# DecodeGenetics/BamQC

Measured on AMD Instinct MI355X. Metric: BAM records/sec (and GB/s vs HBM roofline), 150 bp PE, 1/2/4/8 MI355X, higher is better.
Workload: dtype u8/u32/u64 integer

## Files before the change

bamqc_amd/csrc/bqc_pipeline.cpp:

```cpp
#include "bqc_ctx.h"

#include <algorithm>
#include <chrono>
#include <climits>
#include <cstdlib>
#include <cstring>

#include "../host/parallel.h"

extern "C" {
void bqc_launch_reads_chunks(const DevBatch&, const StateLayout&, uint64_t*, const DevRefs&, uint32_t*, uint32_t grid, uint32_t fast_table, hipStream_t);
void bqc_launch_nm_extra(const DevBatch&, const StateLayout&, uint64_t*, const DevRefs&, uint32_t*, hipStream_t);
void bqc_launch_long(const DevBatch&, const StateLayout&, uint64_t*, const DevRefs&, uint32_t*, uint32_t*, uint32_t max_len_ub, uint32_t max_read_len, uint32_t, uint32_t, uint32_t* t8rows, uint32_t* t8_used, uint32_t t8_lane, uint32_t* cyc_tiles, uint32_t* cyc_used, uint32_t slot_cap, hipStream_t);
uint32_t bqc_long_slots(uint32_t max_len_ub, uint32_t max_read_len, uint32_t n_chunks_ub, uint32_t n_cu);
void bqc_launch_cov(const DevBatch&, const StateLayout&, uint64_t*, uint32_t* carry, uint32_t* parity, const uint8_t* lane_mask, uint8_t* started,
                    const uint8_t* started_after, uint32_t n_lanes, hipStream_t);
void bqc_launch_add_words(uint64_t* state, const uint64_t* idx, const uint64_t* val, uint32_t n, hipStream_t);
void bqc_launch_or_bytes(uint8_t* dst, const uint8_t* src, uint32_t n, hipStream_t);
void bqc_launch_short(const DevBatch&, const StateLayout&, uint64_t*, const DevRefs&, uint32_t*, uint32_t grid, uint32_t* t8rows, uint32_t* t8_used, hipStream_t);
uint32_t bqc_short_parts();
void bqc_launch_t8_fold(const uint32_t* t8rows, const uint32_t* t8_used, uint32_t n_slots, const StateLayout&, uint64_t* state, uint32_t lane, hipStream_t);
void bqc_launch_err_merge(ErrRec* dst, const ErrRec* src, hipStream_t);
void bqc_launch_cov_final(const StateLayout&, uint64_t*, const uint32_t* carry, const uint32_t* parity, const uint8_t* started, const uint8_t* sel, uint32_t count_start, hipStream_t);
}
// ... 338 lines not shown
    Carver cv;
    cv.take(256);
    m.h2d_begin = cv.off;
    const size_t cb[13] = {2 * n, n, n, 4 * n, 4 * n, 4 * n, 4 * n, 4 * n, 4 * n, 2 * n, H.seq_bytes, H.qual_bytes, 4 * H.cigar_words};
    for (int k = 0; k < 13; ++k) { m.col_bytes[k] = in_place ? 0 : cb[k]; m.o_col[k] = cv.take(in_place ? 0 : cb[k] + (k >= 10 ? 512 : 0)); }
    m.o_xr = cv.take(4ull * b->n_nm_extra); m.o_xv = cv.take(4ull * b->n_nm_extra);
    m.o_cov_in = cv.take(in_place ? 0 : sizeof(CovEntry) * n);
    m.o_order = cv.take(H.multi_lane ? 4 * n : 0);
    m.o_sws = cv.take(sizeof(SuperWindow) * H.sws.size());
    m.o_stretch = cv.take(sizeof(Stretch) * H.stretches.size());
    m.o_tiles = cv.take(sizeof(CovTile) * H.tiles.size());
    m.o_mask = cv.take(nl); m.o_started = cv.take(nl);
    m.o_aidx = cv.take(8 * H.add_idx.size()); m.o_aval = cv.take(8 * H.add_val.size());
    m.h2d_end = cv.off;
    const uint64_t nblk = (n + 1023) / 1024, n_sw = H.sws.size(), n_st = H.stretches.size();
    const uint64_t perm_cap = 3 * n + H.cigar_words + 128 * (n_sw + n_st + 1);
    const uint64_t cf_cap = (2 * n + 128 * n_sw) / 256 + H.cigar_words / 256 + 4 * n_st + 16;
    const uint64_t cs_cap = H.n_slow / BQC_CHUNK_READS + n_st + 4;
    const uint64_t cx_cap = H.cigar_words / 2 + 1;
    if (perm_cap > 0xFFFFFFF0ull) return bqc_fail(c, BQC_ERR_ARG, "batch too large (split the batch)");
    const size_t o_flag2 = cv.take(2 * n), o_soff = cv.take(4 * n), o_qoff = cv.take(4 * n), o_cgoff = cv.take(4 * n), o_cov = cv.take(sizeof(CovEntry) * n),
                 o_covx = cv.take(sizeof(CovExtra) * cx_cap), o_cls = cv.take(2 * n), o_segs = cv.take(sizeof(TripSeg) * (H.cigar_words + 1)),
                 o_perm = cv.take(4 * perm_cap), o_cf = cv.take(sizeof(Chunk) * cf_cap), o_cs = cv.take(sizeof(Chunk) * cs_cap),
                 o_desc = cv.take(sizeof(BatchDesc)), o_err = cv.take(sizeof(ErrRec)), o_cursave = cv.take(8), o_bsz = cv.take(24 * nblk), o_btgt = cv.take(8 * nblk),
                 o_bmf = cv.take(8 * nblk), o_swc = cv.take(sizeof(SwCounts) * n_sw), o_swp = cv.take(sizeof(SwPlan) * n_sw),
                 o_rsum = cv.take(H.n_slow ? 12 * n : 0), o_otmp = cv.take(order_on_device && H.multi_lane ? 4 * lane_order_tmp_words((uint32_t)n, nl) : 0);
    const size_t need = cv.off + 256;
    if (m.dcap < need) {
        if (m.dmem) { (void)hipFree(m.dmem); m.dmem = nullptr; m.dcap = 0; }
        if (from_pool)
            for (size_t k = 0; k < c->pool.size(); ++k)
                if (c->pool[k].second >= need && c->pool[k].second <= 2 * need + (64u << 20)) {
                    m.dmem = c->pool[k].first; m.dcap = c->pool[k].second;
                    c->pool.erase(c->pool.begin() + k);
                    break;
                }
        if (!m.dmem) {
            const size_t cap = need + need / 8;
            const hipError_t he = hipMalloc(&m.dmem, cap);
            if (he != hipSuccess) { m.dmem = nullptr; return bqc_fail(c, BQC_ERR_DEVICE, "hipMalloc(%zu) failed: %s", cap, hipGetErrorString(he)); }
            m.dcap = cap;
        }
    }
    char* base = (char*)m.dmem;
    DevBatch& d = m.d;
    d = DevBatch{};
    d.n_reads = (uint32_t)n;
// ... 9 lines not shown
    d.chunks = (const Chunk*)(base + o_cs); d.chunks_fast = (const Chunk*)(base + o_cf);
    d.desc = (const BatchDesc*)(base + o_desc);
    d.nm_extra_read = (const uint32_t*)(base + m.o_xr); d.nm_extra_val = (const int32_t*)(base + m.o_xv); d.n_nm_extra = b->n_nm_extra;
    d.cov = (const CovEntry*)(base + o_cov); d.cov_extra = (const CovExtra*)(base + o_covx);
    d.cov_tiles = (const CovTile*)(base + m.o_tiles); d.n_cov_tiles = (uint32_t)H.tiles.size();
    d.segs = (const TripSeg*)(base + o_segs);
    PrepArgs& p = m.prep;
    p = PrepArgs{};
    p.n = (uint32_t)n; p.n_lanes = nl; p.max_read_len = c->opt.max_read_len; p.no_fast = c->no_fast ? 1u : 0u; p.replay = 0;
    p.flag_in = (const uint16_t*)(base + m.o_col[0]); p.mapq = d.mapq; p.lane = d.lane; p.rid = d.rid; p.pos = d.pos; p.as_ = d.as_;
    p.l_seq = d.l_seq; p.n_cigar = d.n_cigar; p.qual = d.qual; p.cigar = d.cigar;
    p.cov_in = (const CovEntry*)(base + m.o_cov_in); p.order = d.order;
    p.sws = (const SuperWindow*)(base + m.o_sws); p.n_sw = (uint32_t)n_sw;
    p.stretches = (const Stretch*)(base + m.o_stretch); p.n_stretch = (uint32_t)n_st;
    p.fasta_index = c->d_fasta_index;
    p.flag_out = (uint16_t*)(base + o_flag2); p.seq_off = (uint32_t*)(base + o_soff); p.qual_off = (uint32_t*)(base + o_qoff);
    p.cigar_off = (uint32_t*)(base + o_cgoff); p.cov_out = (CovEntry*)(base + o_cov); p.cov_extra = (CovExtra*)(base + o_covx);
    p.cov_extra_cap = (uint32_t)std::min<uint64_t>(cx_cap, 0xFFFFFFFFull); p.cls = (uint16_t*)(base + o_cls); p.segs = (TripSeg*)(base + o_segs);
    p.perm = (uint32_t*)(base + o_perm); p.perm_cap = (uint32_t)perm_cap;
    p.chunks_fast = (Chunk*)(base + o_cf); p.chunks_fast_cap = (uint32_t)cf_cap;
    p.chunks_slow = (Chunk*)(base + o_cs); p.chunks_slow_cap = (uint32_t)cs_cap;
    p.desc = (BatchDesc*)(base + o_desc); p.err = (ErrRec*)(base + o_err);
    p.cursor = c->d_cursor; p.cursor_save = (int32_t*)(base + o_cursave);
    p.blk_sizes = (unsigned long long*)(base + o_bsz); p.blk_tgt = (uint32_t*)(base + o_btgt); p.blk_maxfast = (uint32_t*)(base + o_bmf);
    p.sw_counts = (SwCounts*)(base + o_swc); p.sw_plan = (SwPlan*)(base + o_swp);
    m.d_lane_mask = (uint8_t*)(base + m.o_mask); m.d_started_after = (uint8_t*)(base + m.o_started);
    m.d_add_idx = (uint64_t*)(base + m.o_aidx); m.d_add_val = (uint64_t*)(base + m.o_aval); m.n_add = (uint32_t)H.add_idx.size();
    m.d_rsum = H.n_slow ? (uint32_t*)(base + o_rsum) : nullptr;
    m.d_order_tmp = order_on_device && H.multi_lane ? (uint32_t*)(base + o_otmp) : nullptr;
    m.d_err = p.err;
    m.algo_bytes = 48ull * n + H.seq_bytes + H.qual_bytes + 4 * H.cigar_words;
    m.n_slow = H.n_slow; m.max_len_slow = H.max_len_slow; m.n_chunks_slow_ub = (uint32_t)cs_cap; m.t8_lane = H.t8_lane;
    m.lane_bits[0] = m.lane_bits[1] = m.lane_bits[2] = m.lane_bits[3] = 0;
    for (size_t l = 0; l < H.lane_count.size() && l < 256; ++l) if (H.lane_count[l]) m.lane_bits[l >> 6] |= 1ull << (l & 63);
    if (in_place) {
        d.mapq = b->mapq; d.lane = b->lane; d.rid = b->rid; d.pos = b->pos; d.tlen = b->tlen; d.nm = b->nm; d.as_ = b->as; d.l_seq = b->l_seq; d.n_cigar = b->n_cigar;
        d.seq = b->seq; d.qual = b->qual; d.cigar = b->cigar;
        p.flag_in = b->flag; p.mapq = d.mapq; p.lane = d.lane; p.rid = d.rid; p.pos = d.pos; p.as_ = d.as_; p.l_seq = d.l_seq; p.n_cigar = d.n_cigar; p.qual = d.qual; p.cigar = d.cigar;
        p.cov_in = in_place;
    }
    m.processed = false;
    return 0;
}

static void fill_tables(const BatchMem& m, const bqc_batch* b, const HostPass& H, char* img, size_t img_begin , bool anchors_on_device = false)
{
    auto at = [&](size_t off) { return img + (off - img_begin); };
// ... 665 lines not shown
```

bamqc_amd/csrc/k_prep.hip:

```cpp
#include <algorithm>
#include "kernels_common.h"
#include "prep.h"

#define PR_THREADS 256
#define PR_PER_THREAD 4
#define PR_BLOCK (PR_THREADS * PR_PER_THREAD)

__device__ __forceinline__ uint32_t wave_scan_incl_max(uint32_t v)
{
    v = max(v, (uint32_t)__builtin_amdgcn_update_dpp(0, (int)v, 0x111, 0xF, 0xF, true));
    v = max(v, (uint32_t)__builtin_amdgcn_update_dpp(0, (int)v, 0x112, 0xF, 0xF, true));
    v = max(v, (uint32_t)__builtin_amdgcn_update_dpp(0, (int)v, 0x114, 0xF, 0xF, true));
    v = max(v, (uint32_t)__builtin_amdgcn_update_dpp(0, (int)v, 0x118, 0xF, 0xF, true));
    v = max(v, (uint32_t)__builtin_amdgcn_update_dpp(0, (int)v, 0x142, 0xA, 0xF, false));
    v = max(v, (uint32_t)__builtin_amdgcn_update_dpp(0, (int)v, 0x143, 0xC, 0xF, false));
    return v;
}
__device__ __forceinline__ uint32_t block_scan_excl(uint32_t v, uint32_t* sh, uint32_t* total)
{
    const uint32_t inc = wave_scan_incl(v), w = threadIdx.x >> 6, nw = blockDim.x >> 6;
    block_sync();
    if (lane_id() == WAVE - 1) sh[w] = inc;
    block_sync();
    uint32_t base = 0, tot = 0;
    for (uint32_t k = 0; k < nw; ++k) { const uint32_t x = sh[k]; if (k < w) base += x; tot += x; }
    *total = tot;
    return base + inc - v;
}
__device__ __forceinline__ uint32_t block_scan_excl_max(uint32_t v, uint32_t* sh, uint32_t* total)
{
    const uint32_t inc = wave_scan_incl_max(v), w = threadIdx.x >> 6, nw = blockDim.x >> 6;
    block_sync();
    if (lane_id() == WAVE - 1) sh[w] = inc;
    block_sync();
    uint32_t base = 0, tot = 0;
    for (uint32_t k = 0; k < nw; ++k) { const uint32_t x = sh[k]; if (k < w) base = max(base, x); tot = max(tot, x); }
    *total = tot;
    const uint32_t prev = (uint32_t)__builtin_amdgcn_update_dpp(0, (int)inc, 0x138 , 0xF, 0xF, true);
    return max(base, prev);
}
__device__ __forceinline__ void err_key(ErrRec* e, uint32_t read, uint32_t order)
{
    atomicMin(&e->first_key, ((unsigned long long)read << 3) | order);
}

__global__ __launch_bounds__(PR_THREADS) void k_prep_sizes(PrepArgs a)
{
    __shared__ unsigned long long sh[3 * (PR_THREADS / 64)];
    if (blockIdx.x == 0 && threadIdx.x == 0) {
        a.err->first_key = BQC_ERRKEY_NONE; a.err->flags = 0; a.err->aux0 = a.err->aux1 = 0;
        a.desc->n_cov_extra = 0;
        if (a.pend_extra_n) *a.pend_extra_n = 0;
        if (a.replay) *a.cursor = *a.cursor_save; else *a.cursor_save = *a.cursor;
    }
    for (uint32_t k = blockIdx.x * PR_THREADS + threadIdx.x; k < a.n_sw; k += gridDim.x * PR_THREADS) a.sw_counts[k] = SwCounts{0, 0, 0, 0};
    const uint32_t b0 = blockIdx.x * PR_BLOCK;
    unsigned long long s1 = 0, s2 = 0, s3 = 0;
#pragma unroll
    for (int j = 0; j < PR_PER_THREAD; ++j) {
        const uint32_t i = b0 + j * PR_THREADS + threadIdx.x;
        if (i < a.n) { const uint32_t L = a.l_seq[i]; s1 += (L + 1) / 2; s2 += L; s3 += a.n_cigar[i]; }
    }
#pragma unroll
    for (int o = 32; o > 0; o >>= 1) { s1 += __shfl_xor(s1, o); s2 += __shfl_xor(s2, o); s3 += __shfl_xor(s3, o); }
    if (lane_id() == 0) { const uint32_t w = threadIdx.x >> 6; sh[3 * w] = s1; sh[3 * w + 1] = s2; sh[3 * w + 2] = s3; }
    block_sync();
    if (threadIdx.x < 3) {
        unsigned long long t = 0;
        for (uint32_t w = 0; w < PR_THREADS / 64; ++w) t += sh[3 * w + threadIdx.x];
        a.blk_sizes[3ull * blockIdx.x + threadIdx.x] = t;
    }
}

__global__ __launch_bounds__(1024) void k_prep_scan(PrepArgs a)
{
    __shared__ unsigned long long sh[3 * 1024];
    const uint32_t nblk = (a.n + PR_BLOCK - 1) / PR_BLOCK;
    const uint32_t per = (nblk + blockDim.x - 1) / blockDim.x;
    const uint32_t lo = min(nblk, threadIdx.x * per), hi = min(nblk, lo + per);
    unsigned long long t[3] = {0, 0, 0};
    for (uint32_t b = lo; b < hi; ++b)
        for (int k = 0; k < 3; ++k) t[k] += a.blk_sizes[3ull * b + k];
    for (int k = 0; k < 3; ++k) sh[3 * threadIdx.x + k] = t[k];
    block_sync();
    for (uint32_t d = 1; d < blockDim.x; d <<= 1) {
        unsigned long long v[3] = {0, 0, 0};
        if (threadIdx.x >= d) for (int k = 0; k < 3; ++k) v[k] = sh[3 * (threadIdx.x - d) + k];
        block_sync();
        for (int k = 0; k < 3; ++k) sh[3 * threadIdx.x + k] += v[k];
        block_sync();
    }
    unsigned long long run[3];
    for (int k = 0; k < 3; ++k) run[k] = sh[3 * threadIdx.x + k] - t[k];
    for (uint32_t b = lo; b < hi; ++b) {
        bool over = false;
        for (int k = 0; k < 3; ++k) {
            const unsigned long long s = a.blk_sizes[3ull * b + k];
            a.blk_sizes[3ull * b + k] = run[k];
            run[k] += s;
            over |= run[k] > 0xFFFFFFFFull;
        }
        if (over) err_key(a.err, b * PR_BLOCK, 3);
    }
}

struct CigarView {
    uint32_t w[4];
    const uint32_t* cg;
    __device__ __forceinline__ uint32_t at(uint32_t k) const
    {
        if (k < 4u) return k == 0u ? w[0] : k == 1u ? w[1] : k == 2u ? w[2] : w[3];
        return cg[k];
    }
};
__device__ __forceinline__ int triplet_eligible(uint32_t flag, uint32_t mapq, int32_t as, const CigarView& cv, uint32_t ncig)
{
    if (!(flag & 0x1) || !(flag & 0x2) || (flag & 0x4) || (flag & 0x8) || (flag & 0x100)) return 0;
    if (mapq < 60) return 0;
    if (as == BQC_AS_ABSENT || as < 0) return -1;
    if (as < 50) return 0;
    uint32_t clipped = 0;
    for (uint32_t k = 0; k < ncig; ++k) {
        const uint32_t wd = cv.at(k), op = wd & 15u;
        if (op == 4u || op == 5u) clipped += wd >> 4;
    }
// ... 91 lines not shown
                        a.segs[co + nseg] = TripSeg{i, (int32_t)posv, (uint32_t)ia | ((uint32_t)ib << 8), 0};
                        ++nseg;
                    }
                    rp += nn; cpos += nn;
                }
            }
        }
    }
    o.flag = flag;
    o.ce = ce;
    o.cls = ((fast ? ((flag & 0x40u) ? 0u : 1u) : 2u) << 8) | nseg;
    return o;
}

#ifndef PR_WAVES_PER_EU
#define PR_WAVES_PER_EU 4
#endif
__global__ __launch_bounds__(PR_THREADS) __attribute__((amdgpu_waves_per_eu(PR_WAVES_PER_EU, PR_WAVES_PER_EU))) void k_prep_reads(PrepArgs a, DevRefs refs)
{
    __shared__ uint32_t sh[2 * (PR_THREADS / 64)];
    __shared__ uint32_t red[8];
    const uint32_t i0 = blockIdx.x * PR_BLOCK + 4u * threadIdx.x;
    const unsigned long long gs = a.blk_sizes[3ull * blockIdx.x], gq = a.blk_sizes[3ull * blockIdx.x + 1], gc = a.blk_sizes[3ull * blockIdx.x + 2];
    if (threadIdx.x < 8) red[threadIdx.x] = threadIdx.x == 0 ? 0xFFFFFFFFu : 0u;
    ReadIn in[4];
    const uint32_t nlive = i0 >= a.n ? 0u : min(4u, a.n - i0);
    if (nlive == 4u) {
        const uint4 vl = *(const uint4*)(a.l_seq + i0);
        const uint2 vc = *(const uint2*)(a.n_cigar + i0), vf = *(const uint2*)(a.flag_in + i0);
        const uint32_t vlane = *(const uint32_t*)(a.lane + i0), vmq = *(const uint32_t*)(a.mapq + i0);
        const int4 vr = *(const int4*)(a.rid + i0), vp = *(const int4*)(a.pos + i0), va = *(const int4*)(a.as_ + i0);
        const uint4 c01 = *(const uint4*)(a.cov_in + i0), c23 = *(const uint4*)(a.cov_in + i0 + 2);
        const uint32_t Ls[4] = {vl.x, vl.y, vl.z, vl.w}, ncs[4] = {vc.x & 0xFFFFu, vc.x >> 16, vc.y & 0xFFFFu, vc.y >> 16};
        const uint32_t fs[4] = {vf.x & 0xFFFFu, vf.x >> 16, vf.y & 0xFFFFu, vf.y >> 16};
        const int32_t rs[4] = {vr.x, vr.y, vr.z, vr.w}, ps[4] = {vp.x, vp.y, vp.z, vp.w}, as[4] = {va.x, va.y, va.z, va.w};
        const CovEntry cs[4] = {{c01.x, c01.y}, {c01.z, c01.w}, {c23.x, c23.y}, {c23.z, c23.w}};
#pragma unroll
        for (int j = 0; j < 4; ++j) in[j] = ReadIn{Ls[j], ncs[j], fs[j], (vlane >> (8 * j)) & 0xFFu, (vmq >> (8 * j)) & 0xFFu, rs[j], ps[j], as[j], cs[j]};
    } else {
#pragma unroll
        for (int j = 0; j < 4; ++j) {
            in[j] = ReadIn{0, 0, 0x900u, 0, 0, -1, 0, 0, CovEntry{BQC_COV_NONE, 0}};
            if ((uint32_t)j < nlive) { const uint32_t i = i0 + j; in[j] = ReadIn{a.l_seq[i], a.n_cigar[i], a.flag_in[i], a.lane[i], a.mapq[i], a.rid[i], a.pos[i], a.as_[i], a.cov_in[i]}; }
        }
    }
    uint32_t ls[4], lq[4], lc[4], ts = 0, tq = 0, tc = 0;
#pragma unroll
    for (int j = 0; j < 4; ++j) { ls[j] = ts; lq[j] = tq; lc[j] = tc; ts += (in[j].L + 1) / 2; tq += in[j].L; tc += in[j].nc; }
    uint32_t tot;
    const unsigned long long bs = gs + block_scan_excl(ts, sh, &tot), bq = gq + block_scan_excl(tq, sh, &tot), bc = gc + block_scan_excl(tc, sh, &tot);
    ReadOut out[4];
    CigarView cv[4];
    bool ref_loaded[4];
    int32_t target[4];
    unsigned long long cos[4];
    bool oks[4];
#pragma unroll
    for (int j = 0; j < 4; ++j) {
        const unsigned long long so = bs + ls[j], qo = bq + lq[j], co = bc + lc[j];
        cos[j] = co;
        oks[j] = so + (in[j].L + 1) / 2 <= 0xFFFFFFFFull && qo + in[j].L <= 0xFFFFFFFFull && co + in[j].nc <= 0xFFFFFFFFull;
        const bool live = (uint32_t)j < nlive && oks[j];
        cv[j].cg = a.cigar + (uint32_t)co;
#pragma unroll
        for (uint32_t k = 0; k < 4u; ++k) cv[j].w[k] = live && k < in[j].nc ? cv[j].cg[k] : 0u;
        const int32_t rid = in[j].rid;
        const bool rid_ok = (uint32_t)j < nlive && rid >= 0 && (uint32_t)rid < refs.n_refs;
        ref_loaded[j] = rid_ok && refs.ref[rid] != nullptr;
        target[j] = rid_ok ? (a.fasta_index ? a.fasta_index[rid] : rid) : -1;
    }
    uint32_t tmax = 0, tmin = 0xFFFFFFFFu, maxfast = 0, maxlong = 0, cnt[4] = {0, 0, 0, 0};
    bool local_bad[4] = {false, false, false, false};
#pragma unroll
// ... 53 lines not shown

__global__ __launch_bounds__(PR_THREADS) void k_build_count(PrepArgs a)
{
    __shared__ uint32_t sh[4 * (PR_THREADS / 64)];
    const SuperWindow sw = a.sws[blockIdx.x];
    uint32_t c[4] = {0, 0, 0, 0};
    for (uint32_t p = threadIdx.x; p < sw.count; p += PR_THREADS) {
        const uint32_t r = a.order ? a.order[sw.begin + p] : sw.begin + p;
        uint32_t ns;
        const uint32_t cl = read_class(a, r, &ns);
        c[cl] += 1;
        c[3] += ns;
    }
    for (int k = 0; k < 4; ++k) c[k] = wave_sum(c[k]);
    if (lane_id() == 0) for (int k = 0; k < 4; ++k) sh[4 * (threadIdx.x >> 6) + k] = c[k];
    block_sync();
    if (threadIdx.x < 4) {
        uint32_t t = 0;
        for (uint32_t w = 0; w < PR_THREADS / 64; ++w) t += sh[4 * w + threadIdx.x];
        ((uint32_t*)&a.sw_counts[blockIdx.x])[threadIdx.x] = t;
    }
}

__global__ __launch_bounds__(1024) void k_build_plan(PrepArgs a)
{
    __shared__ uint32_t sh[2 * 16 + 8];
    __shared__ uint32_t s_fast_w, s_first_bad, s_gmin;
    const uint32_t nblk = (a.n + PR_BLOCK - 1) / PR_BLOCK;
    {
        uint32_t carry = (uint32_t)(*a.cursor + 1);
        uint32_t mf = 0, gmin = 0xFFFFFFFFu;
        if (threadIdx.x == 0) { s_first_bad = 0xFFFFFFFFu; s_gmin = 0xFFFFFFFFu; }
        for (uint32_t b0 = 0; b0 < nblk; b0 += blockDim.x) {
            const uint32_t b = b0 + threadIdx.x;
            const uint32_t mx = b < nblk ? a.blk_tgt[2ull * b] : 0u, mn = b < nblk ? a.blk_tgt[2ull * b + 1] : 0xFFFFFFFFu;
            if (b < nblk) mf = max(mf, a.blk_maxfast[2ull * b]);
            uint32_t tot;
            const uint32_t before = max(carry, block_scan_excl_max(mx, sh, &tot));
            gmin = min(gmin, mn);
            if (mn < before) atomicMin(&s_first_bad, b);
            carry = max(carry, tot);
        }
        if (gmin != 0xFFFFFFFFu) atomicMin(&s_gmin, gmin);
        block_sync();
        const uint32_t bad = s_first_bad;
        if (bad != 0xFFFFFFFFu) {
            uint32_t before = (uint32_t)(*a.cursor + 1);
            for (uint32_t b = threadIdx.x; b < bad; b += blockDim.x) before = max(before, a.blk_tgt[2ull * b]);
            uint32_t tot;
            (void)block_scan_excl_max(before, sh, &tot);
            for (uint32_t i = bad * PR_BLOCK + threadIdx.x; i < min(a.n, (bad + 1) * PR_BLOCK); i += blockDim.x)
                if (a.flag_out[i] & BQC_FLAG_TRIPLET) {
                    const int32_t rid = a.rid[i];
                    const uint32_t t1 = (uint32_t)(a.fasta_index ? a.fasta_index[rid] : rid) + 1u;
                    if (t1 < tot) err_key(a.err, i, 5);
                }
        }
        for (int o = 32; o > 0; o >>= 1) mf = max(mf, (uint32_t)__shfl_xor((int)mf, o));
        block_sync();
        if (lane_id() == 0) sh[threadIdx.x >> 6] = mf;
        block_sync();
        if (threadIdx.x == 0) {
            uint32_t m = 0;
            for (uint32_t w = 0; w < blockDim.x / 64; ++w) m = max(m, sh[w]);
            s_fast_w = max(1u, (m + 8 * BQC_FAST_NH - 1) / (8 * BQC_FAST_NH));
            *a.cursor = (int32_t)carry - 1;
            if (a.cursor[1] < 0 && s_gmin != 0xFFFFFFFFu) a.cursor[1] = (int32_t)s_gmin - 1;
        }
        block_sync();
    }
    const uint32_t fast_w = s_fast_w, rpw = 64u / fast_w, h0 = (rpw + 1) / 2, h1 = rpw / 2;
    const uint32_t groups_cap = BQC_FAST_WAVES * (64u / rpw);
    const uint32_t seg_cap = groups_cap * rpw;
    uint32_t run_g = 0, run_q = 0, run_s = 0;
    for (uint32_t s0 = 0; s0 < a.n_sw; s0 += blockDim.x) {
        const uint32_t s = s0 + threadIdx.x;
        uint32_t g = 0, q = 0, sl = 0;
        if (s < a.n_sw) {
            const SwCounts c = a.sw_counts[s];
            g = max((c.n0 + h0 - 1) / h0, (c.n1 + h1 - 1) / h1);
            q = c.n_seg; sl = c.n_slow;
        }
        uint32_t tg, tq, ts;
        const uint32_t eg = run_g + block_scan_excl(g, sh, &tg), eq = run_q + block_scan_excl(q, sh, &tq), es = run_s + block_scan_excl(sl, sh, &ts);
        if (s < a.n_sw) a.sw_plan[s] = SwPlan{eg, g, eq, es};
        run_g += tg; run_q += tq; run_s += ts;
    }
    __threadfence_block();
    block_sync();
    __shared__ uint32_t s_pb, s_cf, s_cs, s_g0, s_q0, s_s0, s_ng, s_nq, s_ns, s_lane, s_sw0, s_sw1, s_longest;
    if (threadIdx.x == 0) { s_pb = 0; s_cf = 0; s_cs = 0; }
    block_sync();
    for (uint32_t st = 0; st < a.n_stretch; ++st) {
        if (threadIdx.x == 0) {
            const Stretch S = a.stretches[st];
            const SwPlan p0 = a.sw_plan[S.sw_begin];
            const SwPlan pl = a.sw_plan[S.sw_end - 1];
            const SwCounts cl = a.sw_counts[S.sw_end - 1];
            s_g0 = p0.group_base; s_q0 = p0.seg_base; s_s0 = p0.slow_base;
            s_ng = pl.group_base + pl.n_groups - p0.group_base;
            s_nq = pl.seg_base + cl.n_seg - p0.seg_base;
            s_ns = pl.slow_base + cl.n_slow - p0.slow_base;
            s_lane = S.lane; s_sw0 = S.sw_begin; s_sw1 = S.sw_end;
        }
        block_sync();
        const uint32_t pb = s_pb, ng = s_ng, nq = s_nq, ns = s_ns, lane = s_lane;
        const uint32_t nq_pad = (nq + rpw - 1) / rpw * rpw;
        const uint32_t seg0 = pb + ng * rpw, slow0 = seg0 + nq_pad;
        for (uint32_t s = s_sw0 + threadIdx.x; s < s_sw1; s += blockDim.x) {
            SwPlan p = a.sw_plan[s];
            p.group_base = pb + (p.group_base - s_g0) * rpw;
            p.seg_base = seg0 + (p.seg_base - s_q0);
            p.slow_base = slow0 + (p.slow_base - s_s0);
            a.sw_plan[s] = p;
        }
        for (uint32_t k = nq + threadIdx.x; k < nq_pad; k += blockDim.x) a.perm[seg0 + k] = 0xFFFFFFFFu;
        const uint32_t n_rc = (ng + groups_cap - 1) / groups_cap, n_sc = (nq_pad + seg_cap - 1) / seg_cap, n_lc = (ns + BQC_CHUNK_READS - 1) / BQC_CHUNK_READS;
        const uint32_t cf = s_cf, cs = s_cs;
        for (uint32_t k = threadIdx.x; k < n_rc; k += blockDim.x) {
            const uint32_t g = min(groups_cap, ng - k * groups_cap);
            if (cf + k < a.chunks_fast_cap) a.chunks_fast[cf + k] = Chunk{pb + k * groups_cap * rpw, g * rpw, lane, g * rpw, 0, 0, 0, 0};
        }
        for (uint32_t k = threadIdx.x; k < n_sc; k += blockDim.x) {
            const uint32_t e = min(seg_cap, nq_pad - k * seg_cap);
            if (cf + n_rc + k < a.chunks_fast_cap) a.chunks_fast[cf + n_rc + k] = Chunk{seg0 + k * seg_cap, e, lane, 0, 0, 0, 0, 0};
        }
        for (uint32_t k = threadIdx.x; k < n_lc; k += blockDim.x) {
            const uint32_t e = min((uint32_t)BQC_CHUNK_READS, ns - k * BQC_CHUNK_READS);
            if (cs + k < a.chunks_slow_cap) a.chunks_slow[cs + k] = Chunk{slow0 + k * BQC_CHUNK_READS, e, lane, 0, 0, 0, 0, 0};
        }
        block_sync();
        if (threadIdx.x == 0) { s_pb = slow0 + ns; s_cf = cf + n_rc + n_sc; s_cs = cs + n_lc; }
        block_sync();
    }
    uint32_t longest = 0;
    for (uint32_t b = threadIdx.x; b < nblk; b += blockDim.x) longest = max(longest, a.blk_maxfast[2ull * b + 1]);
    for (int o = 32; o > 0; o >>= 1) longest = max(longest, (uint32_t)__shfl_xor((int)longest, o));
    if (threadIdx.x == 0) s_longest = 0;
    block_sync();
    if (lane_id() == 0) atomicMax(&s_longest, longest);
    block_sync();
    if (threadIdx.x == 0) {
        if (s_pb > a.perm_cap || s_cf > a.chunks_fast_cap || s_cs > a.chunks_slow_cap) atomicOr(&a.err->flags, BQC_DEVERR_INTERNAL);
        const bool fatal = a.err->first_key != BQC_ERRKEY_NONE || (a.err->flags & BQC_DEVERR_INTERNAL);
        a.desc->fatal = fatal ? 1u : 0u;
        a.desc->n_chunks_fast = fatal ? 0u : min(s_cf, a.chunks_fast_cap);
        a.desc->n_chunks_slow = fatal ? 0u : min(s_cs, a.chunks_slow_cap);
        a.desc->fast_w = fast_w;
        a.desc->n_perm = s_pb;
        a.desc->long_max_len = s_longest;
        if (a.desc->n_cov_extra > a.cov_extra_cap) a.desc->n_cov_extra = a.cov_extra_cap;
        const unsigned long long key = a.err->first_key;
        if (key != BQC_ERRKEY_NONE) {
            const uint32_t i = (uint32_t)(key >> 3), order = (uint32_t)key & 7u;
            if (i < a.n) { a.err->aux0 = order == 1 ? a.l_seq[i] : order == 2 ? a.lane[i] : (uint32_t)a.rid[i]; a.err->aux1 = a.lane[i]; }
        }
    }
}

__device__ __forceinline__ void block_scan_excl4(uint32_t v[4], uint32_t* sh, uint32_t tot[4])
{
    const uint32_t w = threadIdx.x >> 6, nw = blockDim.x >> 6;
    uint32_t inc[4];
#pragma unroll
    for (int k = 0; k < 4; ++k) inc[k] = wave_scan_incl(v[k]);
    block_sync();
    if (lane_id() == WAVE - 1) {
#pragma unroll
        for (int k = 0; k < 4; ++k) sh[4 * w + k] = inc[k];
    }
    block_sync();
#pragma unroll
    for (int k = 0; k < 4; ++k) {
// ... 38 lines not shown
    uint32_t co[SC_PER];
#pragma unroll
    for (int k = 0; k < SC_PER; ++k) co[k] = (v[k] >> 8) < 3u && (v[k] & 0xFFu) ? a.cigar_off[r[k]] : 0u;
    uint32_t tot[4];
    block_scan_excl4(c, sh, tot);
    uint32_t k0 = c[0], k1 = c[1], k2 = c[2], k3 = c[3];
#pragma unroll
    for (int k = 0; k < SC_PER; ++k) {
        const uint32_t cl = v[k] >> 8, ns = v[k] & 0xFFu;
        if (cl == 0u) { ent[(k0 / h0) * rpw + k0 % h0] = r[k]; ++k0; }
        else if (cl == 1u) { ent[(k1 / h1) * rpw + h0 + k1 % h1] = r[k]; ++k1; }
        else if (cl == 2u) a.perm[pl.slow_base + k2++] = r[k];
        if (cl < 3u && ns) { for (uint32_t j = 0; j < ns; ++j) a.perm[pl.seg_base + k3 + j] = BQC_ENTRY_SEG | (co[k] + j); k3 += ns; }
    }
    block_sync();
    for (uint32_t k = threadIdx.x; k < n_ent; k += PR_THREADS) a.perm[pl.group_base + k] = ent[k];
}

extern "C" void bqc_launch_prep(const PrepArgs& a, const DevRefs& refs, hipStream_t s)
{
    if (a.n == 0) return;
    const uint32_t nblk = (a.n + PR_BLOCK - 1) / PR_BLOCK;
    hipLaunchKernelGGL(k_prep_sizes, dim3(nblk), dim3(PR_THREADS), 0, s, a);
    hipLaunchKernelGGL(k_prep_scan, dim3(1), dim3(1024), 0, s, a);
    hipLaunchKernelGGL(k_prep_reads, dim3(nblk), dim3(PR_THREADS), 0, s, a, refs);
    if (a.order) hipLaunchKernelGGL(k_build_count, dim3(a.n_sw), dim3(PR_THREADS), 0, s, a);
    hipLaunchKernelGGL(k_build_plan, dim3(1), dim3(1024), 0, s, a);
    hipLaunchKernelGGL(k_build_scatter, dim3(a.n_sw), dim3(PR_THREADS), 0, s, a);
}

__device__ __forceinline__ uint32_t pend_interval(uint32_t pos, uint32_t c0, uint32_t len)
{
    const uint32_t lo = pos + c0;
    if (!len || lo >= 2u * BQC_VSIZE) return 0u;
    const uint32_t hi = min(lo + len, 2u * BQC_VSIZE);
    return lo | ((hi - lo) << 16);
}
__global__ __launch_bounds__(256) void k_pend_cov(uint32_t n, const CovEntry* __restrict__ cov_in, const PendRun* __restrict__ pend, const PendExtra* __restrict__ extra,
                                                     const uint32_t* __restrict__ extra_n, uint32_t extra_cap, const uint8_t* __restrict__ lane,
                                                     CovEntry* __restrict__ cov_out, CovExtra* __restrict__ cov_extra, BatchDesc* __restrict__ desc)
{
    const uint32_t ne = min(*extra_n, extra_cap);
    for (uint32_t i = blockIdx.x * blockDim.x + threadIdx.x; i < n; i += gridDim.x * blockDim.x) {
        const CovEntry ce = cov_in[i];
        const PendRun r = pend[i];
        cov_out[i] = CovEntry{ce.win, pend_interval(ce.off_len, r.c0, r.len)};
    }
    for (uint32_t e = blockIdx.x * blockDim.x + threadIdx.x; e < ne; e += gridDim.x * blockDim.x) {
        const PendExtra x = extra[e];
        const CovEntry ce = cov_in[x.idx];
// ... 11 lines not shown
```

bamqc_amd/csrc/prep.h:

```cpp
#pragma once
#include <stdint.h>
#include "device_types.h"

struct Stretch {
    uint32_t lane, sw_begin, sw_end, pad;
};

struct PrepArgs {
    uint32_t n;
    uint32_t n_lanes, max_read_len;
    uint32_t no_fast;
    uint32_t replay;
    const uint16_t* flag_in;
    const uint8_t* mapq;
    const uint8_t* lane;
    const int32_t* rid;
    const int32_t* pos;
    const int32_t* as_;
    const uint32_t* l_seq;
    const uint16_t* n_cigar;
    const uint8_t* qual;
    const uint32_t* cigar;
    const CovEntry* cov_in;
    const uint32_t* order;
// ... 6 lines not shown
    uint32_t* seq_off;
    uint32_t* qual_off;
    uint32_t* cigar_off;
    CovEntry* cov_out;
    CovExtra* cov_extra;
    uint32_t cov_extra_cap;
    PendRun* pend;
    PendExtra* pend_extra;
    uint32_t* pend_extra_n;
    uint32_t pend_extra_cap;
    uint16_t* cls;
    TripSeg* segs;
    uint32_t* perm;
    uint32_t perm_cap;
    Chunk* chunks_fast;
    uint32_t chunks_fast_cap;
    Chunk* chunks_slow;
    uint32_t chunks_slow_cap;
    BatchDesc* desc;
    ErrRec* err;
    int32_t* cursor;
    int32_t* cursor_save;
    unsigned long long* blk_sizes;
    uint32_t* blk_tgt;
    uint32_t* blk_maxfast;
    SwCounts* sw_counts;
    SwPlan* sw_plan;
};

extern "C" void bqc_launch_prep(const PrepArgs& a, const DevRefs& refs, hipStream_t s);
extern "C" void bqc_launch_pend_cov(uint32_t n, const CovEntry* cov_in, const PendRun* pend, const PendExtra* extra, const uint32_t* extra_n, uint32_t extra_cap,
                                    const uint8_t* lane, CovEntry* cov_out, CovExtra* cov_extra, BatchDesc* desc, hipStream_t s);
```

Before: 4.400 billion.

## Rework prep scan and build-plan kernels with wave-level DPP scans and per-wave offsets

The per-block size scan in k_prep_sizes now also writes per-wave exclusive offsets (blk_wave). k_prep_reads uses these offsets with a wave-only DPP scan in place of three block-wide scans with barriers. The single-block k_prep_scan swaps its log-step shared-memory scan for a 64-bit DPP wave scan plus a cross-wave combine and batches its loads. k_build_plan gives each thread a contiguous range, computes max/min/longest in one pass with wave scans, and drops the separate longest-read reduction. The aim is fewer barriers and less serial latency in the single-block kernels, at the cost of an extra buffer and more complex error-detection logic.

```diff
diff --git a/bamqc_amd/csrc/bqc_pipeline.cpp b/bamqc_amd/csrc/bqc_pipeline.cpp
--- a/bamqc_amd/csrc/bqc_pipeline.cpp
+++ b/bamqc_amd/csrc/bqc_pipeline.cpp
@@ -384,7 +384,7 @@
     const size_t o_flag2 = cv.take(2 * n), o_soff = cv.take(4 * n), o_qoff = cv.take(4 * n), o_cgoff = cv.take(4 * n), o_cov = cv.take(sizeof(CovEntry) * n),
                  o_covx = cv.take(sizeof(CovExtra) * cx_cap), o_cls = cv.take(2 * n), o_segs = cv.take(sizeof(TripSeg) * (H.cigar_words + 1)),
                  o_perm = cv.take(4 * perm_cap), o_cf = cv.take(sizeof(Chunk) * cf_cap), o_cs = cv.take(sizeof(Chunk) * cs_cap),
-                 o_desc = cv.take(sizeof(BatchDesc)), o_err = cv.take(sizeof(ErrRec)), o_cursave = cv.take(8), o_bsz = cv.take(24 * nblk), o_btgt = cv.take(8 * nblk),
+                 o_desc = cv.take(sizeof(BatchDesc)), o_err = cv.take(sizeof(ErrRec)), o_cursave = cv.take(8), o_bsz = cv.take(24 * nblk), o_bwv = cv.take(64 * nblk), o_btgt = cv.take(8 * nblk),
                  o_bmf = cv.take(8 * nblk), o_swc = cv.take(sizeof(SwCounts) * n_sw), o_swp = cv.take(sizeof(SwPlan) * n_sw),
                  o_rsum = cv.take(H.n_slow ? 12 * n : 0), o_otmp = cv.take(order_on_device && H.multi_lane ? 4 * lane_order_tmp_words((uint32_t)n, nl) : 0);
     const size_t need = cv.off + 256;
@@ -440,7 +440,7 @@
     p.chunks_slow = (Chunk*)(base + o_cs); p.chunks_slow_cap = (uint32_t)cs_cap;
     p.desc = (BatchDesc*)(base + o_desc); p.err = (ErrRec*)(base + o_err);
     p.cursor = c->d_cursor; p.cursor_save = (int32_t*)(base + o_cursave);
-    p.blk_sizes = (unsigned long long*)(base + o_bsz); p.blk_tgt = (uint32_t*)(base + o_btgt); p.blk_maxfast = (uint32_t*)(base + o_bmf);
+    p.blk_sizes = (unsigned long long*)(base + o_bsz); p.blk_wave = (uint32_t*)(base + o_bwv); p.blk_tgt = (uint32_t*)(base + o_btgt); p.blk_maxfast = (uint32_t*)(base + o_bmf);
     p.sw_counts = (SwCounts*)(base + o_swc); p.sw_plan = (SwPlan*)(base + o_swp);
     m.d_lane_mask = (uint8_t*)(base + m.o_mask); m.d_started_after = (uint8_t*)(base + m.o_started);
     m.d_add_idx = (uint64_t*)(base + m.o_aidx); m.d_add_val = (uint64_t*)(base + m.o_aval); m.n_add = (uint32_t)H.add_idx.size();
diff --git a/bamqc_amd/csrc/k_prep.hip b/bamqc_amd/csrc/k_prep.hip
--- a/bamqc_amd/csrc/k_prep.hip
+++ b/bamqc_amd/csrc/k_prep.hip
@@ -16,16 +16,22 @@
     v = max(v, (uint32_t)__builtin_amdgcn_update_dpp(0, (int)v, 0x143, 0xC, 0xF, false));
     return v;
 }
-__device__ __forceinline__ uint32_t block_scan_excl(uint32_t v, uint32_t* sh, uint32_t* total)
-{
-    const uint32_t inc = wave_scan_incl(v), w = threadIdx.x >> 6, nw = blockDim.x >> 6;
-    block_sync();
-    if (lane_id() == WAVE - 1) sh[w] = inc;
-    block_sync();
-    uint32_t base = 0, tot = 0;
-    for (uint32_t k = 0; k < nw; ++k) { const uint32_t x = sh[k]; if (k < w) base += x; tot += x; }
-    *total = tot;
-    return base + inc - v;
+template <int CTRL, int ROW_MASK, bool BOUND_CTRL>
+__device__ __forceinline__ unsigned long long dpp64(unsigned long long v)
+{
+    const uint32_t lo = (uint32_t)__builtin_amdgcn_update_dpp(0, (int)(uint32_t)v, CTRL, ROW_MASK, 0xF, BOUND_CTRL);
+    const uint32_t hi = (uint32_t)__builtin_amdgcn_update_dpp(0, (int)(uint32_t)(v >> 32), CTRL, ROW_MASK, 0xF, BOUND_CTRL);
+    return ((unsigned long long)hi << 32) | lo;
+}
+__device__ __forceinline__ unsigned long long wave_scan_incl64(unsigned long long v)
+{
+    v += dpp64<0x111, 0xF, true>(v);
+    v += dpp64<0x112, 0xF, true>(v);
+    v += dpp64<0x114, 0xF, true>(v);
+    v += dpp64<0x118, 0xF, true>(v);
+    v += dpp64<0x142, 0xA, false>(v);
+    v += dpp64<0x143, 0xC, false>(v);
+    return v;
 }
 __device__ __forceinline__ uint32_t block_scan_excl_max(uint32_t v, uint32_t* sh, uint32_t* total)
 {
@@ -54,13 +60,22 @@
         if (a.replay) *a.cursor = *a.cursor_save; else *a.cursor_save = *a.cursor;
     }
     for (uint32_t k = blockIdx.x * PR_THREADS + threadIdx.x; k < a.n_sw; k += gridDim.x * PR_THREADS) a.sw_counts[k] = SwCounts{0, 0, 0, 0};
-    const uint32_t b0 = blockIdx.x * PR_BLOCK;
+    const uint32_t i0 = blockIdx.x * PR_BLOCK + 4u * threadIdx.x;
+    const uint32_t nlive = i0 >= a.n ? 0u : min(4u, a.n - i0);
+    uint32_t L[4] = {0, 0, 0, 0}, nc[4] = {0, 0, 0, 0};
+    if (nlive == 4u) {
+        const uint4 vl = *(const uint4*)(a.l_seq + i0);
+        const uint2 vc = *(const uint2*)(a.n_cigar + i0);
+        L[0] = vl.x; L[1] = vl.y; L[2] = vl.z; L[3] = vl.w;
+        nc[0] = vc.x & 0xFFFFu; nc[1] = vc.x >> 16; nc[2] = vc.y & 0xFFFFu; nc[3] = vc.y >> 16;
+    } else {
+#pragma unroll
+        for (uint32_t j = 0; j < 4; ++j)
+            if (j < nlive) { L[j] = a.l_seq[i0 + j]; nc[j] = a.n_cigar[i0 + j]; }
+    }
     unsigned long long s1 = 0, s2 = 0, s3 = 0;
 #pragma unroll
-    for (int j = 0; j < PR_PER_THREAD; ++j) {
-        const uint32_t i = b0 + j * PR_THREADS + threadIdx.x;
-        if (i < a.n) { const uint32_t L = a.l_seq[i]; s1 += (L + 1) / 2; s2 += L; s3 += a.n_cigar[i]; }
-    }
+    for (int j = 0; j < 4; ++j) { s1 += (L[j] + 1) / 2; s2 += L[j]; s3 += nc[j]; }
 #pragma unroll
     for (int o = 32; o > 0; o >>= 1) { s1 += __shfl_xor(s1, o); s2 += __shfl_xor(s2, o); s3 += __shfl_xor(s3, o); }
     if (lane_id() == 0) { const uint32_t w = threadIdx.x >> 6; sh[3 * w] = s1; sh[3 * w + 1] = s2; sh[3 * w + 2] = s3; }
@@ -70,37 +85,71 @@
         for (uint32_t w = 0; w < PR_THREADS / 64; ++w) t += sh[3 * w + threadIdx.x];
         a.blk_sizes[3ull * blockIdx.x + threadIdx.x] = t;
     }
-}
-
-__global__ __launch_bounds__(1024) void k_prep_scan(PrepArgs a)
-{
-    __shared__ unsigned long long sh[3 * 1024];
+    if (threadIdx.x < 4 * (PR_THREADS / 64)) {
+        const uint32_t w = threadIdx.x >> 2, k = threadIdx.x & 3u;
+        uint32_t base = 0;
+        if (k < 3u)
+            for (uint32_t q = 0; q < w; ++q) base += (uint32_t)sh[3 * q + k];
+        a.blk_wave[4ull * (PR_THREADS / 64) * blockIdx.x + threadIdx.x] = base;
+    }
+}
+
+#define PS_THREADS 1024
+#define PS_PER 12
+__global__ __launch_bounds__(PS_THREADS) void k_prep_scan(PrepArgs a)
+{
+    __shared__ unsigned long long sh[3 * (PS_THREADS / 64)];
     const uint32_t nblk = (a.n + PR_BLOCK - 1) / PR_BLOCK;
-    const uint32_t per = (nblk + blockDim.x - 1) / blockDim.x;
+    const uint32_t per = (nblk + PS_THREADS - 1) / PS_THREADS;
     const uint32_t lo = min(nblk, threadIdx.x * per), hi = min(nblk, lo + per);
+    unsigned long long* const bsz = a.blk_sizes;
     unsigned long long t[3] = {0, 0, 0};
-    for (uint32_t b = lo; b < hi; ++b)
-        for (int k = 0; k < 3; ++k) t[k] += a.blk_sizes[3ull * b + k];
-    for (int k = 0; k < 3; ++k) sh[3 * threadIdx.x + k] = t[k];
-    block_sync();
-    for (uint32_t d = 1; d < blockDim.x; d <<= 1) {
-        unsigned long long v[3] = {0, 0, 0};
-        if (threadIdx.x >= d) for (int k = 0; k < 3; ++k) v[k] = sh[3 * (threadIdx.x - d) + k];
-        block_sync();
-        for (int k = 0; k < 3; ++k) sh[3 * threadIdx.x + k] += v[k];
-        block_sync();
-    }
+    for (uint32_t b0 = lo; b0 < hi; b0 += PS_PER) {
+        unsigned long long x[PS_PER][3];
+#pragma unroll
+        for (uint32_t j = 0; j < PS_PER; ++j)
+#pragma unroll
+            for (int k = 0; k < 3; ++k) x[j][k] = b0 + j < hi ? bsz[3ull * (b0 + j) + k] : 0ull;
+#pragma unroll
+        for (uint32_t j = 0; j < PS_PER; ++j)
+#pragma unroll
+            for (int k = 0; k < 3; ++k) t[k] += x[j][k];
+    }
+    const uint32_t w = threadIdx.x >> 6;
     unsigned long long run[3];
-    for (int k = 0; k < 3; ++k) run[k] = sh[3 * threadIdx.x + k] - t[k];
-    for (uint32_t b = lo; b < hi; ++b) {
-        bool over = false;
-        for (int k = 0; k < 3; ++k) {
-            const unsigned long long s = a.blk_sizes[3ull * b + k];
-            a.blk_sizes[3ull * b + k] = run[k];
-            run[k] += s;
-            over |= run[k] > 0xFFFFFFFFull;
-        }
-        if (over) err_key(a.err, b * PR_BLOCK, 3);
+#pragma unroll
+    for (int k = 0; k < 3; ++k) run[k] = wave_scan_incl64(t[k]);
+    if (lane_id() == WAVE - 1) {
+#pragma unroll
+        for (int k = 0; k < 3; ++k) sh[3 * w + k] = run[k];
+    }
+    block_sync();
+#pragma unroll
+    for (int k = 0; k < 3; ++k) {
+        unsigned long long base = 0;
+#pragma unroll
+        for (uint32_t q = 0; q < PS_THREADS / 64; ++q) base += q < w ? sh[3 * q + k] : 0ull;
+        run[k] += base - t[k];
+    }
+    bool keyed = false;
+    for (uint32_t b0 = lo; b0 < hi; b0 += PS_PER) {
+        unsigned long long x[PS_PER][3];
+#pragma unroll
+        for (uint32_t j = 0; j < PS_PER; ++j)
+#pragma unroll
+            for (int k = 0; k < 3; ++k) x[j][k] = b0 + j < hi ? bsz[3ull * (b0 + j) + k] : 0ull;
+#pragma unroll
+        for (uint32_t j = 0; j < PS_PER; ++j) {
+            if (b0 + j >= hi) break;
+            bool over = false;
+#pragma unroll
+            for (int k = 0; k < 3; ++k) {
+                bsz[3ull * (b0 + j) + k] = run[k];
+                run[k] += x[j][k];
+                over |= run[k] > 0xFFFFFFFFull;
+            }
+            if (over && !keyed) { err_key(a.err, (b0 + j) * PR_BLOCK, 3); keyed = true; }
+        }
     }
 }
 
@@ -238,6 +287,8 @@
     __shared__ uint32_t red[8];
     const uint32_t i0 = blockIdx.x * PR_BLOCK + 4u * threadIdx.x;
     const unsigned long long gs = a.blk_sizes[3ull * blockIdx.x], gq = a.blk_sizes[3ull * blockIdx.x + 1], gc = a.blk_sizes[3ull * blockIdx.x + 2];
+    const uint32_t wv = __builtin_amdgcn_readfirstlane(threadIdx.x >> 6);
+    const uint4 wb = *(const uint4*)(a.blk_wave + 4ull * (PR_THREADS / 64) * blockIdx.x + 4u * wv);
     if (threadIdx.x < 8) red[threadIdx.x] = threadIdx.x == 0 ? 0xFFFFFFFFu : 0u;
     ReadIn in[4];
     const uint32_t nlive = i0 >= a.n ? 0u : min(4u, a.n - i0);
@@ -263,8 +314,8 @@
     uint32_t ls[4], lq[4], lc[4], ts = 0, tq = 0, tc = 0;
 #pragma unroll
     for (int j = 0; j < 4; ++j) { ls[j] = ts; lq[j] = tq; lc[j] = tc; ts += (in[j].L + 1) / 2; tq += in[j].L; tc += in[j].nc; }
-    uint32_t tot;
-    const unsigned long long bs = gs + block_scan_excl(ts, sh, &tot), bq = gq + block_scan_excl(tq, sh, &tot), bc = gc + block_scan_excl(tc, sh, &tot);
+    const unsigned long long bs = gs + (uint32_t)(wb.x + wave_scan_incl(ts) - ts), bq = gq + (uint32_t)(wb.y + wave_scan_incl(tq) - tq),
+                             bc = gc + (uint32_t)(wb.z + wave_scan_incl(tc) - tc);
     ReadOut out[4];
     CigarView cv[4];
     bool ref_loaded[4];
@@ -364,73 +415,110 @@
     }
 }
 
-__global__ __launch_bounds__(1024) void k_build_plan(PrepArgs a)
-{
-    __shared__ uint32_t sh[2 * 16 + 8];
-    __shared__ uint32_t s_fast_w, s_first_bad, s_gmin;
-    const uint32_t nblk = (a.n + PR_BLOCK - 1) / PR_BLOCK;
+#define BP_THREADS 1024
+#define BP_WAVES (BP_THREADS / 64)
+#define BP_PER 12
+#define BP_SW 4
+__global__ __launch_bounds__(BP_THREADS) void k_build_plan(PrepArgs a)
+{
+    __shared__ uint32_t sh[4 * BP_WAVES];
+    __shared__ uint32_t sg[3 * BP_WAVES];
+    __shared__ uint32_t s_first_bad;
+    const uint32_t nblk = (a.n + PR_BLOCK - 1) / PR_BLOCK, w = threadIdx.x >> 6;
+    if (threadIdx.x == 0) s_first_bad = 0xFFFFFFFFu;
+    const uint32_t cur1 = (uint32_t)(*a.cursor + 1);
+    const uint32_t sper = (a.n_sw + BP_THREADS - 1) / BP_THREADS, slo = min(a.n_sw, threadIdx.x * sper), shi = min(a.n_sw, slo + sper);
+    SwCounts swc[BP_SW];
+#pragma unroll
+    for (uint32_t j = 0; j < BP_SW; ++j) swc[j] = slo + j < shi ? a.sw_counts[slo + j] : SwCounts{0, 0, 0, 0};
+    const uint32_t per = (nblk + BP_THREADS - 1) / BP_THREADS, lo = min(nblk, threadIdx.x * per), hi = min(nblk, lo + per);
+    uint32_t tmx = 0, tmn = 0xFFFFFFFFu, mf = 0, ml = 0;
+    bool bad = false;
+    for (uint32_t b0 = lo; b0 < hi; b0 += BP_PER) {
+        uint2 t[BP_PER], m[BP_PER];
+#pragma unroll
+        for (uint32_t j = 0; j < BP_PER; ++j) {
+            const bool in = b0 + j < hi;
+            t[j] = in ? *(const uint2*)(a.blk_tgt + 2ull * (b0 + j)) : make_uint2(0u, 0xFFFFFFFFu);
+            m[j] = in ? *(const uint2*)(a.blk_maxfast + 2ull * (b0 + j)) : make_uint2(0u, 0u);
+        }
+#pragma unroll
+        for (uint32_t j = 0; j < BP_PER; ++j) {
+            bad |= t[j].y < tmx;
+            tmx = max(tmx, t[j].x); tmn = min(tmn, t[j].y); mf = max(mf, m[j].x); ml = max(ml, m[j].y);
+        }
+    }
+    const uint32_t inc = wave_scan_incl_max(tmx);
     {
-        uint32_t carry = (uint32_t)(*a.cursor + 1);
-        uint32_t mf = 0, gmin = 0xFFFFFFFFu;
-        if (threadIdx.x == 0) { s_first_bad = 0xFFFFFFFFu; s_gmin = 0xFFFFFFFFu; }
-        for (uint32_t b0 = 0; b0 < nblk; b0 += blockDim.x) {
-            const uint32_t b = b0 + threadIdx.x;
-            const uint32_t mx = b < nblk ? a.blk_tgt[2ull * b] : 0u, mn = b < nblk ? a.blk_tgt[2ull * b + 1] : 0xFFFFFFFFu;
-            if (b < nblk) mf = max(mf, a.blk_maxfast[2ull * b]);
-            uint32_t tot;
-            const uint32_t before = max(carry, block_scan_excl_max(mx, sh, &tot));
-            gmin = min(gmin, mn);
-            if (mn < before) atomicMin(&s_first_bad, b);
-            carry = max(carry, tot);
-        }
-        if (gmin != 0xFFFFFFFFu) atomicMin(&s_gmin, gmin);
-        block_sync();
-        const uint32_t bad = s_first_bad;
-        if (bad != 0xFFFFFFFFu) {
-            uint32_t before = (uint32_t)(*a.cursor + 1);
-            for (uint32_t b = threadIdx.x; b < bad; b += blockDim.x) before = max(before, a.blk_tgt[2ull * b]);
-            uint32_t tot;
-            (void)block_scan_excl_max(before, sh, &tot);
-            for (uint32_t i = bad * PR_BLOCK + threadIdx.x; i < min(a.n, (bad + 1) * PR_BLOCK); i += blockDim.x)
-                if (a.flag_out[i] & BQC_FLAG_TRIPLET) {
-                    const int32_t rid = a.rid[i];
-                    const uint32_t t1 = (uint32_t)(a.fasta_index ? a.fasta_index[rid] : rid) + 1u;
-                    if (t1 < tot) err_key(a.err, i, 5);
-                }
-        }
-        for (int o = 32; o > 0; o >>= 1) mf = max(mf, (uint32_t)__shfl_xor((int)mf, o));
-        block_sync();
-        if (lane_id() == 0) sh[threadIdx.x >> 6] = mf;
-        block_sync();
-        if (threadIdx.x == 0) {
-            uint32_t m = 0;
-            for (uint32_t w = 0; w < blockDim.x / 64; ++w) m = max(m, sh[w]);
-            s_fast_w = max(1u, (m + 8 * BQC_FAST_NH - 1) / (8 * BQC_FAST_NH));
-            *a.cursor = (int32_t)carry - 1;
-            if (a.cursor[1] < 0 && s_gmin != 0xFFFFFFFFu) a.cursor[1] = (int32_t)s_gmin - 1;
-        }
-        block_sync();
-    }
-    const uint32_t fast_w = s_fast_w, rpw = 64u / fast_w, h0 = (rpw + 1) / 2, h1 = rpw / 2;
+        const uint32_t imn = wave_scan_incl_max(~tmn), imf = wave_scan_incl_max(mf), iml = wave_scan_incl_max(ml);
+        if (lane_id() == WAVE - 1) { sh[4 * w] = inc; sh[4 * w + 1] = imn; sh[4 * w + 2] = imf; sh[4 * w + 3] = iml; }
+    }
+    block_sync();
+    uint32_t before = max(cur1, (uint32_t)__builtin_amdgcn_update_dpp(0, (int)inc, 0x138 , 0xF, 0xF, true));
+    uint32_t all_mx = 0, all_nmn = 0, all_mf = 0, all_ml = 0;
+#pragma unroll
+    for (uint32_t q = 0; q < BP_WAVES; ++q) {
+        const uint32_t x = sh[4 * q];
+        if (q < w) before = max(before, x);
+        all_mx = max(all_mx, x); all_nmn = max(all_nmn, sh[4 * q + 1]); all_mf = max(all_mf, sh[4 * q + 2]); all_ml = max(all_ml, sh[4 * q + 3]);
+    }
+    if (bad || tmn < before) {
+        uint32_t bf = before;
+        for (uint32_t b = lo; b < hi; ++b) {
+            const uint2 t = *(const uint2*)(a.blk_tgt + 2ull * b);
+            if (t.y < bf) { atomicMin(&s_first_bad, b); break; }
+            bf = max(bf, t.x);
+        }
+    }
+    block_sync();
+    const uint32_t first_bad = s_first_bad;
+    if (first_bad != 0xFFFFFFFFu) {
+        uint32_t bf = cur1;
+        for (uint32_t b = threadIdx.x; b < first_bad; b += blockDim.x) bf = max(bf, a.blk_tgt[2ull * b]);
+        uint32_t tot;
+        (void)block_scan_excl_max(bf, sh, &tot);
+        for (uint32_t i = first_bad * PR_BLOCK + threadIdx.x; i < min(a.n, (first_bad + 1) * PR_BLOCK); i += blockDim.x)
+            if (a.flag_out[i] & BQC_FLAG_TRIPLET) {
+                const int32_t rid = a.rid[i];
+                const uint32_t t1 = (uint32_t)(a.fasta_index ? a.fasta_index[rid] : rid) + 1u;
+                if (t1 < tot) err_key(a.err, i, 5);
+            }
+    }
+    if (threadIdx.x == 0) {
+        *a.cursor = (int32_t)max(cur1, all_mx) - 1;
+        if (a.cursor[1] < 0 && all_nmn != 0u) a.cursor[1] = (int32_t)~all_nmn - 1;
+    }
+    const uint32_t fast_w = max(1u, (all_mf + 8 * BQC_FAST_NH - 1) / (8 * BQC_FAST_NH)), rpw = 64u / fast_w, h0 = (rpw + 1) / 2, h1 = rpw / 2;
     const uint32_t groups_cap = BQC_FAST_WAVES * (64u / rpw);
     const uint32_t seg_cap = groups_cap * rpw;
-    uint32_t run_g = 0, run_q = 0, run_s = 0;
-    for (uint32_t s0 = 0; s0 < a.n_sw; s0 += blockDim.x) {
-        const uint32_t s = s0 + threadIdx.x;
-        uint32_t g = 0, q = 0, sl = 0;
-        if (s < a.n_sw) {
-            const SwCounts c = a.sw_counts[s];
-            g = max((c.n0 + h0 - 1) / h0, (c.n1 + h1 - 1) / h1);
-            q = c.n_seg; sl = c.n_slow;
-        }
-        uint32_t tg, tq, ts;
-        const uint32_t eg = run_g + block_scan_excl(g, sh, &tg), eq = run_q + block_scan_excl(q, sh, &tq), es = run_s + block_scan_excl(sl, sh, &ts);
-        if (s < a.n_sw) a.sw_plan[s] = SwPlan{eg, g, eq, es};
-        run_g += tg; run_q += tq; run_s += ts;
+    auto n_groups = [&](const SwCounts& c) { return max((c.n0 + h0 - 1) / h0, (c.n1 + h1 - 1) / h1); };
+    uint32_t tg = 0, tq = 0, ts = 0;
+#pragma unroll
+    for (uint32_t j = 0; j < BP_SW; ++j) { tg += n_groups(swc[j]); tq += swc[j].n_seg; ts += swc[j].n_slow; }
+    for (uint32_t s = slo + BP_SW; s < shi; ++s) { const SwCounts c = a.sw_counts[s]; tg += n_groups(c); tq += c.n_seg; ts += c.n_slow; }
+    uint32_t eg = wave_scan_incl(tg), eq = wave_scan_incl(tq), es = wave_scan_incl(ts);
+    if (lane_id() == WAVE - 1) { sg[3 * w] = eg; sg[3 * w + 1] = eq; sg[3 * w + 2] = es; }
+    block_sync();
+    eg -= tg; eq -= tq; es -= ts;
+#pragma unroll
+    for (uint32_t q = 0; q < BP_WAVES; ++q)
+        if (q < w) { eg += sg[3 * q]; eq += sg[3 * q + 1]; es += sg[3 * q + 2]; }
+#pragma unroll
+    for (uint32_t j = 0; j < BP_SW; ++j)
+        if (slo + j < shi) {
+            const uint32_t g = n_groups(swc[j]);
+            a.sw_plan[slo + j] = SwPlan{eg, g, eq, es};
+            eg += g; eq += swc[j].n_seg; es += swc[j].n_slow;
+        }
+    for (uint32_t s = slo + BP_SW; s < shi; ++s) {
+        const SwCounts c = a.sw_counts[s];
+        const uint32_t g = n_groups(c);
+        a.sw_plan[s] = SwPlan{eg, g, eq, es};
+        eg += g; eq += c.n_seg; es += c.n_slow;
     }
     __threadfence_block();
     block_sync();
-    __shared__ uint32_t s_pb, s_cf, s_cs, s_g0, s_q0, s_s0, s_ng, s_nq, s_ns, s_lane, s_sw0, s_sw1, s_longest;
+    __shared__ uint32_t s_pb, s_cf, s_cs, s_g0, s_q0, s_s0, s_ng, s_nq, s_ns, s_lane, s_sw0, s_sw1;
     if (threadIdx.x == 0) { s_pb = 0; s_cf = 0; s_cs = 0; }
     block_sync();
     for (uint32_t st = 0; st < a.n_stretch; ++st) {
@@ -475,13 +563,6 @@
         if (threadIdx.x == 0) { s_pb = slow0 + ns; s_cf = cf + n_rc + n_sc; s_cs = cs + n_lc; }
         block_sync();
     }
-    uint32_t longest = 0;
-    for (uint32_t b = threadIdx.x; b < nblk; b += blockDim.x) longest = max(longest, a.blk_maxfast[2ull * b + 1]);
-    for (int o = 32; o > 0; o >>= 1) longest = max(longest, (uint32_t)__shfl_xor((int)longest, o));
-    if (threadIdx.x == 0) s_longest = 0;
-    block_sync();
-    if (lane_id() == 0) atomicMax(&s_longest, longest);
-    block_sync();
     if (threadIdx.x == 0) {
         if (s_pb > a.perm_cap || s_cf > a.chunks_fast_cap || s_cs > a.chunks_slow_cap) atomicOr(&a.err->flags, BQC_DEVERR_INTERNAL);
         const bool fatal = a.err->first_key != BQC_ERRKEY_NONE || (a.err->flags & BQC_DEVERR_INTERNAL);
@@ -490,7 +571,7 @@
         a.desc->n_chunks_slow = fatal ? 0u : min(s_cs, a.chunks_slow_cap);
         a.desc->fast_w = fast_w;
         a.desc->n_perm = s_pb;
-        a.desc->long_max_len = s_longest;
+        a.desc->long_max_len = all_ml;
         if (a.desc->n_cov_extra > a.cov_extra_cap) a.desc->n_cov_extra = a.cov_extra_cap;
         const unsigned long long key = a.err->first_key;
         if (key != BQC_ERRKEY_NONE) {
@@ -575,10 +656,10 @@
     if (a.n == 0) return;
     const uint32_t nblk = (a.n + PR_BLOCK - 1) / PR_BLOCK;
     hipLaunchKernelGGL(k_prep_sizes, dim3(nblk), dim3(PR_THREADS), 0, s, a);
-    hipLaunchKernelGGL(k_prep_scan, dim3(1), dim3(1024), 0, s, a);
+    hipLaunchKernelGGL(k_prep_scan, dim3(1), dim3(PS_THREADS), 0, s, a);
     hipLaunchKernelGGL(k_prep_reads, dim3(nblk), dim3(PR_THREADS), 0, s, a, refs);
     if (a.order) hipLaunchKernelGGL(k_build_count, dim3(a.n_sw), dim3(PR_THREADS), 0, s, a);
-    hipLaunchKernelGGL(k_build_plan, dim3(1), dim3(1024), 0, s, a);
+    hipLaunchKernelGGL(k_build_plan, dim3(1), dim3(BP_THREADS), 0, s, a);
     hipLaunchKernelGGL(k_build_scatter, dim3(a.n_sw), dim3(PR_THREADS), 0, s, a);
 }
 
diff --git a/bamqc_amd/csrc/prep.h b/bamqc_amd/csrc/prep.h
--- a/bamqc_amd/csrc/prep.h
+++ b/bamqc_amd/csrc/prep.h
@@ -52,6 +52,7 @@
     int32_t* cursor;
     int32_t* cursor_save;
     unsigned long long* blk_sizes;
+    uint32_t* blk_wave;
     uint32_t* blk_tgt;
     uint32_t* blk_maxfast;
     SwCounts* sw_counts;
```

Result: faster. 4.456 billion, median of 6 (+1.3%).
